# hojinYang/spotify_recSys_challenge_2018

Measured on AMD Instinct MI355X. Metric: playlists scored/sec (encode+decode+top-500) at |vocab|~170k, higher is better.
Workload: dtype f32; 1 GPU; untied DAE scoring: encode+decode(all 170000 cols)+top-500 over 140000 track cols, hidden=256, batch=256/GPU (global 256), ids=zipf, b_dec=zipf, BASELINE.json configs[1]; vocab=170000, n_tracks=140000, hidden=256, global_batch=256, k=500, parallelism=1 GPU, streams=3, decode_gate=True, tau_exchange=False

## Files before the change

include/dae_hip.h:

```cpp
#ifndef DAE_HIP_H
#define DAE_HIP_H

#include <stddef.h>
#include <stdint.h>

#ifdef __cplusplus
extern "C" {
#endif

typedef struct dae_ctx dae_ctx;

#define DAE_OK            0
#define DAE_ERR_ARG      -1
#define DAE_ERR_HIP      -2
#define DAE_ERR_NOMEM    -3
#define DAE_ERR_STATE    -4

#define DAE_OUT_SCORE     0
#define DAE_OUT_LOGIT     1

#define DAE_DTYPE_F32     0
#define DAE_DTYPE_BF16    1
#define DAE_DTYPE_BF16_EXACT 2

// ... 97 lines not shown
                   int k, int out_kind,
                   float* out_score, int32_t* out_idx);

int dae_score_topk_begin(dae_ctx* ctx,
                         const int32_t* row_ptr, const int32_t* col, const float* val,
                         const float* W_enc, const float* b_enc,
                         int V, int H, int B, int dtype, int n_tracks,
                         const int32_t* seed_row_ptr, int k, float* tau_out);
int dae_score_topk_finish(dae_ctx* ctx, const float* tau,
                          const int32_t* seed_row_ptr, const int32_t* seed_col,
                          int out_kind, float* out_score, int32_t* out_idx);

int dae_topk_dense(dae_ctx* ctx, const float* logits, int64_t ld, int B, int ncols, int col_base,
                   const int32_t* seed_row_ptr, const int32_t* seed_col,
                   int k, int out_kind, float* out_score, int32_t* out_idx);

int dae_topk_merge(dae_ctx* ctx, int G, int B, int k,
                   const float* cand_logit, const int32_t* cand_idx,
                   int out_kind, float* out_score, int32_t* out_idx);

int dae_set_overlap_hint(dae_ctx* ctx, int batches_in_flight);

int dae_set_decode_gate(dae_ctx* ctx, void* wait_event, void* record_event);

typedef struct dae_pipeline dae_pipeline;
#define DAE_PIPE_BUSY 1
int dae_pipeline_create(int device, const float* W_enc, const float* b_enc, const float* W_dec, const float* b_dec,
                        int V, int H, int n_tracks, int dtype, int k, int group_rows, int64_t max_nnz, int lanes,
                        int want_scores, int result_blocks, dae_pipeline** out);
int dae_pipeline_destroy(dae_pipeline* p);
int dae_pipeline_submit(dae_pipeline* p, const int64_t* positions, const float* values, int values_broadcast, int64_t nnz,
                        int n_rows, uint64_t* ticket_out);
int dae_pipeline_create_titled(int device, const float* W_enc, const float* b_enc, const float* W_dec, const float* b_dec,
                               int V, int H, int n_tracks, const float* emb, int n_char, int E, const float* conv_w,
                               const float* conv_b, const int32_t* filter_sizes, int n_sizes, int F, const float* Output_WT,
                               const float* Output_b, int ld_feat, int L, int dtype, int k, int group_rows, int64_t max_nnz,
                               int lanes, int want_scores, int result_blocks, dae_pipeline** out);
int dae_pipeline_submit_titled(dae_pipeline* p, const int64_t* positions, const float* values, int values_broadcast, int64_t nnz,
                               int n_rows, const int32_t* titles, const float* titles_use, uint64_t* ticket_out);
int dae_pipeline_flush(dae_pipeline* p);
int dae_pipeline_poll(dae_pipeline* p, int wait, uint64_t* ticket, const int32_t** idx, const float** score, int* n_rows,
                      int* block);
int dae_pipeline_release(dae_pipeline* p, int block);
int dae_pipeline_stats(dae_pipeline* p, uint64_t out3[3]);
int dae_pipeline_times(dae_pipeline* p, uint64_t out4[4]);
int dae_pipeline_exact_margin(dae_pipeline* p, float scale);
// ... 173 lines not shown
```

spotify_recsys_challenge_2018_amd/_lib.py:

```python
import ctypes
import os

_HERE = os.path.dirname(os.path.abspath(__file__))
LIB_PATH = os.path.join(_HERE, "libdae_hip.so")

DAE_OUT_SCORE, DAE_OUT_LOGIT = 0, 1
DAE_MAX_K, DAE_MAX_K_DEEP = 1024, 4096
DAE_DTYPE_F32, DAE_DTYPE_BF16, DAE_DTYPE_BF16_EXACT = 0, 1, 2
DAE_CAND_CHUNK = 256

EXPORTS = [
    "dae_version", "dae_create", "dae_destroy", "dae_set_stream", "dae_last_error",
    "dae_scratch_bytes", "dae_profile_enable", "dae_profile_read", "dae_profile_kernel", "dae_clock_probe", "dae_last_plan",
    "dae_coo_to_csr", "dae_seeds_from_csr", "dae_train_set_create", "dae_train_set_destroy", "dae_train_batch", "dae_train_set_attach_titles", "dae_train_titles", "dae_encode", "dae_prepack_decoder", "dae_prepack_decoder_rows", "dae_share_decoder", "dae_exact_bounds",
    "dae_exact_guard_read", "dae_exact_guard_words", "dae_exact_guard_snapshot", "dae_exact_stats_read", "dae_set_exact_margin", "dae_set_exact_margin_range", "dae_set_exact_audit", "dae_exact_audit_read",
    "dae_set_filter_skip", "dae_filter_skip_read", "dae_filter_skip_last", "dae_tile_bounds_read", "dae_sample_skip_read", "dae_live_proof_read", "dae_last_tau_read", "dae_decode_dense", "dae_decode_topk",
    "dae_score_topk", "dae_score_topk_begin", "dae_score_topk_finish", "dae_topk_dense", "dae_topk_merge", "dae_set_train_dtype", "dae_train_forward_backward",
    "dae_train_shard_encode", "dae_train_shard_decode", "dae_train_shard_finish", "dae_title_features", "dae_title_prepack_features",
    "dae_mix_scores", "dae_decode_mix_term", "dae_set_score_mix", "dae_decode_mix_term_add", "dae_ensemble_topk", "dae_mix_topk_exact", "dae_mix_exact_shape_ok", "dae_title_score_exact", "dae_title_score", "dae_row_sums", "dae_mix_weights", "dae_title_loss_backward", "dae_title_loss_backward_cols", "dae_title_conv_backward", "dae_adam_step",
    "dae_adam_rows_begin", "dae_adam_rows_apply", "dae_adam_rows_flush", "dae_set_enc_grad_prezeroed",
    "dae_arm_decoder_adam", "dae_set_decode_gate", "dae_set_overlap_hint",
    "dae_pipeline_create", "dae_pipeline_create_titled", "dae_pipeline_destroy", "dae_pipeline_submit", "dae_pipeline_submit_titled", "dae_pipeline_flush", "dae_pipeline_poll",
    "dae_pipeline_release", "dae_pipeline_stats", "dae_pipeline_exact_margin", "dae_pipeline_times", "dae_pipeline_last_error",
    "dae_rank_metrics", "dae_pipeline_enable_eval", "dae_pipeline_submit_eval", "dae_pipeline_poll_eval",
    "dae_decode_candidates", "dae_score_candidates", "dae_mix_candidates", "dae_rank_candidates",
    "dae_rank_of_plan", "dae_decode_rank_of", "dae_score_rank_of", "dae_mix_rank_of",
    "dae_catalogue_create", "dae_catalogue_destroy", "dae_prepack_decoder_catalogue", "dae_score_topk_catalogue",
    "dae_decode_topk_catalogue", "dae_title_score_catalogue", "dae_pipeline_set_catalogue",
]
DAE_PIPE_BUSY = 1

_lib = None


class DaeError(RuntimeError):
    pass


def load():
    global _lib
    if _lib is not None:
        return _lib
    if not os.path.exists(LIB_PATH):
        raise DaeError(
# ... 71 lines not shown
    lib.dae_decode_mix_term_add.argtypes = lib.dae_decode_mix_term.argtypes
    lib.dae_ensemble_topk.argtypes = [ctypes.POINTER(vp), c_int, ctypes.POINTER(vp), ctypes.POINTER(c_int), ctypes.POINTER(vp),
                                      vp, vp, c_int, vp, c_int, c_int, c_int, vp, vp, c_int, vp, vp]
    lib.dae_mix_topk_exact.argtypes = [vp, vp, vp, c_i64, vp, c_i64, c_int, vp, vp, c_int, vp, vp, c_int, vp, vp, vp]
    lib.dae_mix_exact_shape_ok.argtypes = [c_int, c_int]
    lib.dae_row_sums.argtypes = [vp, vp, vp, vp, c_int, c_f, c_u32, vp]
    lib.dae_title_score_exact.argtypes = [vp, vp, vp, vp, c_int, c_i64, c_int, c_int, vp, vp, c_int, vp, c_int, vp, c_int, c_int, vp, vp,
                                          ctypes.POINTER(ctypes.c_int32), c_int, c_int, c_int, vp, c_int, c_int, vp, vp, vp, vp]
    lib.dae_mix_weights.argtypes = [vp, vp, vp, vp, c_int, c_f, c_u32, vp, vp, vp]
    lib.dae_title_loss_backward.argtypes = [vp, vp, c_i64, vp, c_i64, vp, vp, vp, vp, vp, c_int, c_int, c_int,
                                            vp, c_int, vp, vp, vp, vp, vp]
    lib.dae_title_loss_backward_cols.argtypes = [vp, vp, c_i64, vp, c_i64, vp, vp, vp, vp, vp, c_int, c_int, c_int, c_int,
                                                 vp, c_int, vp, vp, vp, vp, vp]
    lib.dae_title_conv_backward.argtypes = [vp, vp, c_int, c_int, vp, c_int, c_int, vp, ctypes.POINTER(ctypes.c_int32),
                                            c_int, c_int, vp, vp, vp, c_i64, c_f, c_u32, vp, vp, vp]
    lib.dae_adam_step.argtypes = [vp, vp, vp, vp, vp, c_i64, c_f, c_f, c_f, c_f, c_int]
    lib.dae_adam_rows_begin.argtypes = [vp, vp, vp, vp, vp, vp, c_int, c_int, c_int, vp, vp, c_int, c_f, c_f, c_f, c_int]
    lib.dae_adam_rows_apply.argtypes = [vp, vp, vp, vp, vp, vp, vp, c_int, c_int, c_int, vp, vp, c_int,
                                        c_f, c_f, c_f, c_f, c_int]
    lib.dae_adam_rows_flush.argtypes = [vp, vp, vp, vp, vp, vp, c_int, c_int, c_int, c_f, c_f, c_f, c_int]
    lib.dae_set_enc_grad_prezeroed.argtypes = [vp, c_int]
    lib.dae_arm_decoder_adam.argtypes = [vp, vp, vp, c_f, c_f, c_f, c_f, c_int]
    lib.dae_set_decode_gate.argtypes = [vp, vp, vp]
    lib.dae_set_overlap_hint.argtypes = [vp, c_int]
    u64p, i32pp, f32pp, ip = (ctypes.POINTER(ctypes.c_uint64), ctypes.POINTER(ctypes.POINTER(ctypes.c_int32)),
                              ctypes.POINTER(ctypes.POINTER(ctypes.c_float)), ctypes.POINTER(c_int))
    lib.dae_pipeline_create.argtypes = [c_int, vp, vp, vp, vp, c_int, c_int, c_int, c_int, c_int, c_int, c_i64, c_int, c_int, c_int,
                                        ctypes.POINTER(vp)]
    i32p = ctypes.POINTER(ctypes.c_int32)
    lib.dae_pipeline_create_titled.argtypes = ([c_int, vp, vp, vp, vp, c_int, c_int, c_int,
                                                vp, c_int, c_int, vp, vp, i32p, c_int, c_int,
                                                vp, vp, c_int, c_int] +
                                               [c_int] * 3 + [c_i64] + [c_int] * 3 + [ctypes.POINTER(vp)])
    lib.dae_pipeline_submit_titled.argtypes = [vp, vp, vp, c_int, c_i64, c_int, vp, vp, u64p]
    lib.dae_title_score.argtypes = [vp, vp, c_int, vp, vp, c_int, c_i64, c_int, c_int, vp, vp, c_int, vp, c_int, vp, c_int, c_int, vp, vp,
                                    i32p, c_int, c_int, c_int, vp, c_int, c_int, vp, vp, vp, vp]
    lib.dae_pipeline_destroy.argtypes = [vp]
    lib.dae_pipeline_submit.argtypes = [vp, vp, vp, c_int, c_i64, c_int, u64p]
    lib.dae_pipeline_flush.argtypes = [vp]
    lib.dae_pipeline_poll.argtypes = [vp, c_int, u64p, i32pp, f32pp, ip, ip]
    lib.dae_pipeline_release.argtypes = [vp, c_int]
    lib.dae_pipeline_stats.argtypes = [vp, u64p]
    lib.dae_pipeline_exact_margin.argtypes = [vp, c_f]
    lib.dae_pipeline_times.argtypes = [vp, u64p]
    lib.dae_pipeline_last_error.argtypes = [vp]
    lib.dae_rank_metrics.argtypes = [vp, vp, c_i64, c_int, c_int, vp, vp, vp, vp]
# ... 197 lines not shown
        return "f32" if int(dtype) == DAE_DTYPE_F32 else "bf16"

    def _drop_share(self, dtype):
        self.__dict__.setdefault("_shares", {}).pop(self._slot(dtype), None)

    def prepack_decoder_rows(self, W_rows, b_rows, col_lo, dtype=DAE_DTYPE_F32):
        n, H = W_rows.shape
        assert W_rows.is_contiguous() and b_rows.is_contiguous() and b_rows.numel() == n
        self.check(self.lib.dae_prepack_decoder_rows(self.h, _ptr(W_rows), _ptr(b_rows), int(n), H, int(col_lo), int(dtype)))
        self._drop_share(dtype)

    def title_loss_backward_cols(self, z_title, dae_score, y_csr, w_title, w_playlist, col_lo, col_hi, n_batch, feat,
                                 Output_WT_rows, gOutput_WT_rows, gOutput_b_rows, dfeat_partial, cost_partial):
        B, ld = feat.shape
        self.check(self.lib.dae_title_loss_backward_cols(
            self.h, _ptr(z_title), int(z_title.stride(0)), _ptr(dae_score), int(dae_score.stride(0)),
            _ptr(y_csr[0]), _ptr(y_csr[1]), _ptr(y_csr[2]), _ptr(w_title), _ptr(w_playlist), int(B), int(col_lo), int(col_hi),
            int(n_batch), _ptr(feat), int(ld), _ptr(Output_WT_rows), _ptr(gOutput_WT_rows), _ptr(gOutput_b_rows),
            _ptr(dfeat_partial), _ptr(cost_partial)))

    def set_overlap_hint(self, batches_in_flight):
        self.check(self.lib.dae_set_overlap_hint(self.h, int(batches_in_flight)))

    def share_decoder(self, src, dtype=DAE_DTYPE_F32):
        self.check(self.lib.dae_share_decoder(self.h, src.h, int(dtype)))
        self.__dict__.setdefault("_shares", {})[self._slot(dtype)] = src

    def exact_bounds(self, eps_out):
        self.check(self.lib.dae_exact_bounds(self.h, _ptr(eps_out)))

    def set_exact_margin(self, scale):
        self.check(self.lib.dae_set_exact_margin(self.h, float(scale)))
        self._exact_margin = float(scale)

    def set_exact_margin_range(self, col_from, col_to, scale):
        self.check(self.lib.dae_set_exact_margin_range(self.h, int(col_from), int(col_to), float(scale)))

    def set_exact_audit(self, every_n, n_tiles=16):
        self.check(self.lib.dae_set_exact_audit(self.h, int(every_n), int(n_tiles)))

    def exact_audit_read(self):
        a = (ctypes.c_uint64 * 3)()
        self.check(self.lib.dae_exact_audit_read(self.h, a))
        return {"audits": int(a[0]), "checked": int(a[1]), "violations": int(a[2])}

    def exact_guard_read(self):
# ... 540 lines not shown
```

spotify_recsys_challenge_2018_amd/csrc/api.hip:

```cpp
#include <stdarg.h>

#include <climits>

#include "dae_internal.h"

thread_local std::string g_dae_create_err;

int dae_fail(dae_ctx* ctx, int code, const char* fmt, ...)
{
    char buf[512];
    va_list ap;
    va_start(ap, fmt);
    vsnprintf(buf, sizeof(buf), fmt, ap);
    va_end(ap);
    if (ctx) ctx->err = buf; else g_dae_create_err = buf;
    return code;
}

int dae_reserve(dae_ctx* ctx, dae_buf& b, size_t bytes)
{
    if (bytes <= b.bytes && b.p) return DAE_OK;
    if (bytes == 0) bytes = 16;
    if (b.p) {
        hipError_t e = hipStreamSynchronize(ctx->stream);
// ... 24 lines not shown
extern "C" {

int dae_version(void) { return 1002; }

int dae_create(int device, dae_ctx** out)
{
    if (!out) return dae_fail(nullptr, DAE_ERR_ARG, "out is null");
    int n = 0;
    hipError_t e = hipGetDeviceCount(&n);
    if (e != hipSuccess || n <= 0)
        return dae_fail(nullptr, DAE_ERR_HIP, "no HIP device available (%s)", hipGetErrorString(e));
    if (device < 0 || device >= n)
        return dae_fail(nullptr, DAE_ERR_ARG, "device %d out of range [0,%d)", device, n);
    e = hipSetDevice(device);
    if (e != hipSuccess) return dae_fail(nullptr, DAE_ERR_HIP, "hipSetDevice: %s", hipGetErrorString(e));
    hipDeviceProp_t prop;
    e = hipGetDeviceProperties(&prop, device);
    if (e != hipSuccess) return dae_fail(nullptr, DAE_ERR_HIP, "hipGetDeviceProperties: %s", hipGetErrorString(e));
    if (strncmp(prop.gcnArchName, "gfx950", 6) != 0)
        return dae_fail(nullptr, DAE_ERR_HIP, "device %d is %s; this library is built for gfx950 only",
                        device, prop.gcnArchName);
    dae_ctx* c = new dae_ctx();
    c->device = device;
    *out = c;
    return DAE_OK;
}

int dae_destroy(dae_ctx* ctx)
{
    if (!ctx) return DAE_OK;
    (void)hipSetDevice(ctx->device);
    (void)hipStreamSynchronize(ctx->stream);
    auto release = [](dae_buf& b) { if (b.p) (void)hipFree(b.p); };
    for (dae_packed* pk : {&ctx->pk_f32, &ctx->pk_bf16}) {
        if (!pk->borrowed) dae_packed_shared_bufs(*pk, release);
        release(pk->order); release(pk->ident);
    }
    for (dae_buf* b : {&ctx->h_packed, &ctx->sample, &ctx->tau, &ctx->sample_top, &ctx->cand, &ctx->cand_cnt, &ctx->gmax,
                       &ctx->h_packed16, &ctx->h_scratch, &ctx->train_a, &ctx->train_b, &ctx->train_c, &ctx->train_d, &ctx->csr_tmp,
                       &ctx->feed_tmp, &ctx->row_bad, &ctx->guard, &ctx->refined, &ctx->refstat, &ctx->mix_fhat, &ctx->title_scratch,
                       &ctx->tile_band, &ctx->title_tab, &ctx->audit, &ctx->audit_stat, &ctx->title_y1, &ctx->live, &ctx->skip_stat, &ctx->live_sync,
                       &ctx->row_d, &ctx->samp_tab, &ctx->sskip_stat,
                       &ctx->cand_list, &ctx->cat_seeds, &ctx->rank_of})
        release(*b);
    for (hipEvent_t ev : ctx->prof_ev) (void)hipEventDestroy(ev);
    delete ctx;
    return DAE_OK;
}

int dae_set_stream(dae_ctx* ctx, void* hip_stream)
{
    if (!ctx) return DAE_ERR_ARG;
    ctx->stream = static_cast<hipStream_t>(hip_stream);
    return DAE_OK;
}

const char* dae_last_error(const dae_ctx* ctx)
{
    return ctx ? ctx->err.c_str() : g_dae_create_err.c_str();
}

size_t dae_scratch_bytes(const dae_ctx* ctx) { return ctx ? ctx->scratch_total : 0; }

int dae_profile_enable(dae_ctx* ctx, int on)
{
    if (!ctx) return DAE_ERR_ARG;
    ctx->prof_on = on != 0;
    ctx->prof_used = 0;
// ... 95 lines not shown
    if (!pk.borrowed) return;
    dae_packed_shared_bufs(pk, [](dae_buf& b) { b = dae_buf{}; });
    pk.borrowed = false; pk.valid = false; pk.exact = false; pk.order_nrank = -1;
}

int dae_share_decoder(dae_ctx* dst, const dae_ctx* src, int dtype)
{
    if (!dst) return DAE_ERR_ARG;
    if (!src || src == dst) return dae_fail(dst, DAE_ERR_ARG, "dae_share_decoder: needs another context");
    if (dst->device != src->device) return dae_fail(dst, DAE_ERR_ARG, "dae_share_decoder: contexts on different devices");
    if (!dae_known_dtype(dtype)) return dae_fail(dst, DAE_ERR_ARG, "unknown dtype %d", dtype);
    const dae_packed& sp = dtype == DAE_DTYPE_F32 ? src->pk_f32 : src->pk_bf16;
    dae_packed& dp = dtype == DAE_DTYPE_F32 ? dst->pk_f32 : dst->pk_bf16;
    if (!sp.valid || (dtype == DAE_DTYPE_BF16_EXACT && !sp.exact))
        return dae_fail(dst, DAE_ERR_STATE, "dae_share_decoder: the source context holds no such image");
    if (sp.borrowed) return dae_fail(dst, DAE_ERR_ARG, "dae_share_decoder: share from the context that owns the image");
    if (!dp.borrowed) {
        hipError_t e = hipStreamSynchronize(dst->stream);
        if (e != hipSuccess) return dae_fail(dst, DAE_ERR_HIP, "sync: %s", hipGetErrorString(e));
        dae_packed_shared_bufs(dp, [&](dae_buf& b) {
            if (b.p) { (void)hipFree(b.p); dst->scratch_total -= b.bytes; b = dae_buf{}; }
        });
    }
    const dae_buf order = dp.order, ident = dp.ident;
    dp = sp;
    dp.order = order; dp.ident = ident; dp.order_nrank = -1; dp.order_nsamp = -1;
    dp.borrowed = true;
    int rc = dae_reserve(dst, dp.ident, (size_t)(dp.ntiles > 0 ? dp.ntiles : 1) * sizeof(int));
    if (rc) return rc;
    return dae_launch_tile_iota(dst, static_cast<int*>(dp.ident.p), dp.ntiles);
}

int dae_prepack_decoder(dae_ctx* ctx, const float* W_dec, const float* b_dec, int V, int H,
                        int col_lo, int col_hi, int dtype)
{
    if (!ctx) return DAE_ERR_ARG;
    if (!W_dec || !b_dec) return dae_fail(ctx, DAE_ERR_ARG, "null pointer");
    if (H <= 0 || V <= 0 || col_lo < 0 || col_hi > V || col_lo >= col_hi)
        return dae_fail(ctx, DAE_ERR_ARG, "bad shape V=%d H=%d cols=[%d,%d)", V, H, col_lo, col_hi);
    unborrow(dtype == DAE_DTYPE_F32 ? ctx->pk_f32 : ctx->pk_bf16);
    if (dtype == DAE_DTYPE_F32) return dae_launch_prepack_f32(ctx, W_dec, b_dec, V, H, col_lo, col_hi);
    if (dtype == DAE_DTYPE_BF16) return dae_launch_prepack_bf16(ctx, W_dec, b_dec, V, H, col_lo, col_hi);
    if (dtype == DAE_DTYPE_BF16_EXACT) return dae_launch_prepack_bf16(ctx, W_dec, b_dec, V, H, col_lo, col_hi, 1);
    return dae_fail(ctx, DAE_ERR_ARG, "unknown dtype %d", dtype);
}

int dae_prepack_decoder_rows(dae_ctx* ctx, const float* W_rows, const float* b_rows, int n_rows, int H, int col_lo,
                             int dtype)
{
    if (!ctx) return DAE_ERR_ARG;
    if (!W_rows || !b_rows) return dae_fail(ctx, DAE_ERR_ARG, "null pointer");
    if (n_rows <= 0 || H <= 0 || col_lo < 0 || (int64_t)col_lo + n_rows > INT_MAX)
        return dae_fail(ctx, DAE_ERR_ARG, "bad shape n_rows=%d H=%d col_lo=%d", n_rows, H, col_lo);
    const float* W = W_rows - (size_t)col_lo * H;
    const float* b = b_rows - (size_t)col_lo;
    return dae_prepack_decoder(ctx, W, b, col_lo + n_rows, H, col_lo, col_lo + n_rows, dtype);
}

int dae_exact_bounds(dae_ctx* ctx, float* eps_out)
{
    if (!ctx) return DAE_ERR_ARG;
    if (!eps_out) return dae_fail(ctx, DAE_ERR_ARG, "null pointer");
    const dae_packed& pk = ctx->pk_bf16;
// ... 364 lines not shown
                            float keep_prob, uint32_t seed, float* g_emb, float* g_conv_w, float* g_conv_b)
{
    if (!ctx) return DAE_ERR_ARG;
    if (!titles || !emb || !conv_w || !filter_sizes || !argmax || !feat_raw || !dfeat || !g_emb || !g_conv_w || !g_conv_b)
        return dae_fail(ctx, DAE_ERR_ARG, "null pointer");
    if (B <= 0) return DAE_OK;
    if (!(keep_prob > 0.f && keep_prob <= 1.f)) return dae_fail(ctx, DAE_ERR_ARG, "keep probability must be in (0,1]");
    return dae_launch_title_conv_backward(ctx, titles, B, L, emb, n_char, E, conv_w, filter_sizes, n_sizes, F, argmax,
                                          feat_raw, dfeat, ld, keep_prob, seed, g_emb, g_conv_w, g_conv_b);
}

int dae_set_overlap_hint(dae_ctx* ctx, int batches_in_flight)
{
    if (!ctx) return DAE_ERR_ARG;
    ctx->overlap_hint = batches_in_flight > 1 ? 1 : 0;
    return DAE_OK;
}

int dae_set_decode_gate(dae_ctx* ctx, void* wait_event, void* record_event)
{
    if (!ctx) return DAE_ERR_ARG;
    ctx->gate_wait = static_cast<hipEvent_t>(wait_event);
    ctx->gate_record = static_cast<hipEvent_t>(record_event);
    return DAE_OK;
}

int dae_set_enc_grad_prezeroed(dae_ctx* ctx, int on)
{
    if (!ctx) return DAE_ERR_ARG;
    ctx->enc_grad_prezeroed = on ? 1 : 0;
    return DAE_OK;
}

}
```

spotify_recsys_challenge_2018_amd/csrc/dae_internal.h:

```cpp
#pragma once
#include <hip/hip_runtime.h>
#include <hip/hip_ext.h>
#include <stdint.h>
#include <stdio.h>
#include <stdlib.h>
#include <string.h>
#include <string>
#include <unordered_set>
#include <vector>

#include "../../include/dae_hip.h"
#include "score_plan.h"
#include "mix_plan.h"
#include "tau_search.h"
#include "empty_proof.h"

constexpr int DAE_TITLE_MAX_SIZES = 8;
constexpr int DAE_VT = 32;
constexpr int DAE_HPAD = 32;
constexpr int DAE_REFINED_CAP = 4096;
constexpr size_t DAE_GUARD_BYTES = 2 * sizeof(int);

struct dae_buf {
    void* p = nullptr;
    size_t bytes = 0;
};

struct dae_packed {
    bool valid = false;
    bool borrowed = false;
    int V = 0, H = 0, Hp = 0;
    int col_lo = 0, col_hi = 0;
    int ntiles = 0;
    dae_buf W;
    dae_buf bias;
    dae_buf tile_ub; bool ub_valid = false;
    dae_buf bias16;
    dae_buf order;
// ... 36 lines not shown
    hipStream_t stream = nullptr;
    std::string err;
    size_t scratch_total = 0;

    dae_packed pk_f32, pk_bf16;

    dae_buf h_packed;
    dae_buf h_packed16;
    dae_buf h_scratch;
    long long h_geom_key = -1;
    void* h_geom_ptr = nullptr;
    long long h16_geom_key = -1;
    void* h16_geom_ptr = nullptr;
    dae_buf sample;
    dae_buf gmax;
    dae_buf tau;
    dae_buf sample_top;
    dae_buf cand;
    dae_buf cand_cnt;
    dae_buf train_a, train_b, train_c, train_d;
    float* arm_m = nullptr; float* arm_v = nullptr; float arm_alpha = 0.f, arm_b1 = 0.f, arm_b2 = 0.f, arm_eps = 0.f;
    const float* mixT = nullptr; int64_t mix_ld = 0; const float* mix_w = nullptr; int mix_ncols = 0;
    hipEvent_t gate_wait = nullptr, gate_record = nullptr;
    int enc_grad_prezeroed = 0;
    int adam_t = 0; float adam_b1 = 0.f, adam_b2 = 0.f, adam_b1p = 1.f, adam_b2p = 1.f;
    int train_dtype = DAE_DTYPE_F32;
    dae_buf csr_tmp;
    dae_buf feed_tmp;
    dae_topk_state tk;
    int overlap_hint = 0;
    dae_buf row_bad;
    dae_buf refined;
    dae_buf refstat; int refstat_rows = 0;
    dae_buf guard;
    float exact_margin = 1.0f;
    int margin_lo = 0, margin_hi = 0; float margin_scale = 1.0f;
    int audit_every = 64, audit_tiles = 16;
    uint64_t audit_seq = 0, audits_run = 0;
    dae_buf title_y1;
    dae_buf audit_stat;
    dae_buf audit;
    dae_buf mix_fhat;
    dae_buf title_scratch;
    dae_buf title_tab; const float* ttab_emb = nullptr; const float* ttab_w = nullptr; int ttab_nchar = 0, ttab_E = 0, ttab_F = 0,
        ttab_nsizes = 0; int ttab_fs[DAE_TITLE_MAX_SIZES] = {0};
    dae_buf tile_band; long long band_gen = -1; int band_nsamp = 0, band_nbrg = 0, band_waves = 0;
// ... 152 lines not shown
    int mode;
    const int* list;
};
constexpr int DAE_SSKIP_SLOTS = 2 * DAE_NUM_CU;
constexpr int DAE_SSKIP_PAIRS = DAE_SSKIP_SLOTS / DAE_NUM_XCD;
struct dae_sample_skip {
    const float2* ub;
    const float* beta; int n_beta;
    const float* mu;
    const float* row_d;
    const int32_t* seed_row_ptr; int k;
    unsigned long long* stat;
    unsigned* tab;
    float2* pair;
};
int dae_launch_decode_dense_f32(dae_ctx* ctx, const dae_rowgeom& g, int B, const dae_tileset& ts,
                                int apply_sigmoid, int mask_from_col, float* out, int64_t ld,
                                int fill_pad, int dtype = DAE_DTYPE_F32, float* gmax = nullptr,
                                int64_t ld_gmax = 0, int gmax_per_wave = 0, int bias_sel = 0,
                                const dae_sample_skip* skip = nullptr);
int dae_launch_decode_filter_f32(dae_ctx* ctx, const dae_rowgeom& g, int B, const dae_tileset& ts,
                                 const float* tau, int n_valid_col, uint2* cand, int* cand_cnt,
                                 int cap, int dtype = DAE_DTYPE_F32, int bias_sel = 0, const int* live_cnt = nullptr,
                                 const int* live_list = nullptr);

int dae_launch_decode_scaled_T(dae_ctx* ctx, const dae_rowgeom& g, int B, const dae_tileset& ts, const float* row_scale,
                               float* outT, int64_t ldT, int dtype = DAE_DTYPE_F32, bool add = false);

int dae_launch_decode_loss_f32(dae_ctx* ctx, const dae_rowgeom& g, int B, float inv_n_batch,
                               float* dzT, int64_t ldT, float* loss_part, int dtype = DAE_DTYPE_F32,
                               int dz16 = 0);

int dae_launch_decode_loss_rowmajor(dae_ctx* ctx, const dae_rowgeom& g, int B, int V, int H, const float* W,
                                    const float* bias, const float* h, float inv_n_batch, float* dzT, int64_t ldT,
                                    float* loss_part);

int dae_launch_decode_loss_dh(dae_ctx* ctx, const dae_rowgeom& g, int B, int V, int H, const float* W, const float* bias,
                              const float* h, float inv_n_batch, float* dzT, int64_t ldT, float* loss_part, float* part, int Bpad64);

struct dae_decp;
int dae_launch_decode_generic(dae_ctx* ctx, int epi, int dt, const dae_rowgeom& g, const dae_decp& p);
int dae_launch_decode_gmax_half(dae_ctx* ctx, const dae_rowgeom& g, const dae_decp& p);

int dae_train_step_f32(dae_ctx* ctx,
        const int32_t* x_row_ptr, const int32_t* x_col, const float* x_val,
        const int32_t* y_row_ptr, const int32_t* y_col, const float* y_val,
        const float* W_enc, const float* b_enc, const float* W_dec, const float* b_dec,
// ... 174 lines not shown
```

spotify_recsys_challenge_2018_amd/csrc/decode_common.h:

```cpp
#pragma once
#include "dae_internal.h"

typedef float f32x16 __attribute__((ext_vector_type(16)));
typedef __bf16 bf16x8 __attribute__((ext_vector_type(8)));
typedef float f32x2_t __attribute__((ext_vector_type(2)));
typedef __bf16 bf16x2_t __attribute__((ext_vector_type(2)));

template <int N> struct IntC { static constexpr int value = N; };

__device__ __forceinline__ bf16x8 as_bf16x8(const uint4 u) { return __builtin_bit_cast(bf16x8, u); }

__device__ __forceinline__ float dae_bf16_value(float f) { return __uint_as_float(dae_bf16_rne(f) << 16); }

__device__ __forceinline__ unsigned pk_bf16(float a, float b)
{
    const f32x2_t v = {a, b};
    return __builtin_bit_cast(unsigned, __builtin_convertvector(v, bf16x2_t));
}

constexpr int DT_F32 = 0;
constexpr int DT_BF16 = 1;

__device__ __forceinline__ uint4 bf16_ones_fragment(int hi)
{
// ... 1 lines not shown
}

constexpr int EPI_DENSE = 0;
constexpr int EPI_FILTER = 1;
constexpr int EPI_LOSS = 2;
constexpr int EPI_GMAX = 3;
constexpr int EPI_TERM_ADD = 4;

struct dae_decp {
    const float4* Wp;
    const float* bias;
    const uint4* bias16;
    const float4* hp;
    int G;
    int ncols;
    int col_lo;
    int B, n_rg, nb_rg, Bpad;
    dae_tileset ts;
    float* out; int64_t ld; int apply_sigmoid; int mask_from_col; int fill_pad; int vec_ok;
    float* gmax; int64_t ld_gmax;
    int gmax_per_wave;
    const float* tau; int n_valid_col; uint2* cand; int* cand_cnt; int cap;
    const int* live_cnt; const int* live_list;
    dae_sample_skip sk;
    float* outT; int64_t ld_outT; const float* row_scale;
    const float* mixT; int64_t mix_ld; const float* mix_w; int mix_ncols;
    float inv_nb; float* dzT; int64_t ldT; float* loss_part;
    int dz16;
};

template <class T>
__device__ __forceinline__ T dae_max_nan(T a, T b) { return (a != a) ? a : ((b > a || b != b) ? b : a); }
template <class T>
__device__ __forceinline__ T dae_min_nan(T a, T b) { return -dae_max_nan(-a, -b); }

__device__ __forceinline__ bool dae_tile_is_live(float A_t, float M_t, double d_max, float tau_min)
{
    const double d = d_max * (1.0 + 0x1p-40);
    const double A = (double)A_t, dm = d * (double)M_t;
    const double U = A + dm + (fabs(A) + fabs(dm)) * 0x1p-48;
    return !(U < (double)tau_min);
}

__device__ __forceinline__ void dae_edge_tile_bound(const float* tile_ub, int ntiles, int nrank, int lane, float& ea, float& em)
{
    const int t_edge = nrank >> 5;
// ... 38 lines not shown
```

spotify_recsys_challenge_2018_amd/csrc/decode_f32.hip:

```cpp
#include <climits>

#include "decode_common.h"

namespace {

struct LossRmP {
    const float* W; const float* bias; const float* h;
    int V, H, B, n_rg, nb_rg;
    float inv_nb; float* dzT; int64_t ldT; float* loss_part;
};

__global__ __launch_bounds__(512, 1) void decode_loss_dh_bf16_kernel(const LossRmP p, float* __restrict__ part, int Bpad64)
{
    constexpr int NW = 8, LDW = 132, LDT = 18;
    extern __shared__ __attribute__((aligned(16))) unsigned dyn[];
    unsigned* const wt = dyn;
    unsigned* const wt2 = dyn + 2 * 32 * LDW;
    uint4* const hq = reinterpret_cast<uint4*>(dyn + 2 * 32 * LDW + 2 * 256 * LDT);
    float* const wsum = reinterpret_cast<float*>(hq + 8 * 8 * 64);
    const int tid = threadIdx.x, lane = tid & 63, hi = lane >> 5, j = lane & 31;
    const int wave = __builtin_amdgcn_readfirstlane(tid >> 6);
    const int row = wave * 32 + j;
    const int H4 = p.H >> 2;
    const float4* W4 = reinterpret_cast<const float4*>(p.W);
// ... 293 lines not shown
}
#undef K5F_LOAD
#undef K5F_STAGE

template <int DUMMY>
__global__ __launch_bounds__(256, 1) void decode_f32_h256_filter_kernel(const dae_decp p)
{
    constexpr int RB = 4, G = 32, NW = 4, R_TILE = 128;
    extern __shared__ __attribute__((aligned(16))) float4 lds4[];
    const int tid = threadIdx.x;
    const int lane = tid & 63;
    const int wave = __builtin_amdgcn_readfirstlane(tid >> 6);
    const int hi = lane >> 5;
    const int j = lane & 31;

    const int gs = DAE_NUM_XCD * p.n_rg;
    const int q = blockIdx.x / gs, rem_b = blockIdx.x % gs;
    const int rg = rem_b / DAE_NUM_XCD;
    const int bir = q * DAE_NUM_XCD + (rem_b % DAE_NUM_XCD);

    constexpr int n_h4 = RB * 64 * G;
    const int* const tlist = p.live_cnt ? p.live_list + (size_t)rg * p.ts.n_items : p.ts.list;
    const int n_items = p.live_cnt ? __builtin_amdgcn_readfirstlane(p.live_cnt[rg]) : p.ts.n_items;
    if (n_items <= 0) {
        if (tid < R_TILE) p.cand_cnt[(size_t)bir * p.Bpad + rg * R_TILE + tid] = 0;
        return;
    }
    const int n_ws = p.nb_rg * NW;
    const int ws = wave * p.nb_rg + bir;
    const int R = n_items / n_ws, rem = n_items - R * n_ws;
    const bool split = rem > 0 && 2 * rem <= n_ws;
    const int n_it = R + (ws < (split ? 2 * rem : rem) ? 1 : 0);
    auto item_at = [&](int r) {
        r = r < n_it - 1 ? r : n_it - 1;
        r = r < 0 ? 0 : r;
        const int it = r < R ? ws + r * n_ws : R * n_ws + (split ? (ws >> 1) : ws);
        return it < n_items ? it : 0;
    };
    const int tv_cur = tlist[item_at(0)], tv_nxt = tlist[item_at(1)];
    {
        const float4* src = p.hp + (size_t)rg * n_h4;
        constexpr int NT = NW * 64;
#pragma unroll
        for (int i0 = 0; i0 < n_h4; i0 += 8 * NT) {
            float4 v[8];
#pragma unroll
            for (int u = 0; u < 8; ++u) v[u] = src[i0 + u * NT + tid];
#pragma unroll
            for (int u = 0; u < 8; ++u) lds4[i0 + u * NT + tid] = v[u];
        }
    }
    int* lcnt = reinterpret_cast<int*>(lds4 + n_h4);
    float* ltau = reinterpret_cast<float*>(lcnt + R_TILE);
    if (tid < R_TILE) {
        lcnt[tid] = 0;
        ltau[tid] = rg * R_TILE + tid < p.B ? p.tau[rg * R_TILE + tid] : __builtin_inff();
    }
    float4 wb0, wb1, wb2, wb3;
    float4 bA[RB], bB[RB];
    int t_cur = __builtin_amdgcn_readfirstlane(tv_cur), t_nxt = __builtin_amdgcn_readfirstlane(tv_nxt);
    {
        const float4* w0 = p.Wp + (size_t)t_cur * G * 64 + lane;
        wb0 = w0[0]; wb1 = w0[64]; wb2 = w0[128]; wb3 = w0[192];
    }
    __syncthreads();

    float tau_r[RB];
#pragma unroll
    for (int rb = 0; rb < RB; ++rb) tau_r[rb] = ltau[rb * 32 + j];
#pragma unroll
    for (int rb = 0; rb < RB; ++rb) bA[rb] = lds4[rb * 64 + lane];

    for (int r = 0; r < n_it; ++r) {
        const int t = t_cur;
// ... 566 lines not shown
    p.inv_nb = inv_n_batch; p.dzT = dzT; p.ldT = ldT; p.loss_part = loss_part;
    const size_t lds = ((size_t)2 * 32 * 132 + (size_t)2 * 256 * 18) * 4 + (size_t)8 * 8 * 64 * 16 + 64;
    DAE_HIP_CHECK(ctx, dae_lds_limit_once(ctx, &decode_loss_dh_bf16_kernel, lds));
    hipLaunchKernelGGL(decode_loss_dh_bf16_kernel, dim3(g.grid), dim3(512), lds, ctx->stream, p, part, Bpad64);
    DAE_CHECK_LAUNCH(ctx, "decode_loss_dh_bf16_kernel");
    return DAE_OK;
}

int dae_launch_decode_loss_f32(dae_ctx* ctx, const dae_rowgeom& g, int B, float inv_n_batch,
                               float* dzT, int64_t ldT, float* loss_part, int dtype, int dz16)
{
    dae_decp p;
    const dae_packed& pk = dtype == DAE_DTYPE_F32 ? ctx->pk_f32 : ctx->pk_bf16;
    dae_tileset ts{pk.ntiles, 1, 0, static_cast<const int*>(pk.ident.p)};
    int rc = fill_common(ctx, g, B, ts, p, dtype);
    if (rc) return rc;
    p.dzT = dzT; p.ldT = ldT; p.loss_part = loss_part; p.inv_nb = inv_n_batch;
    p.dz16 = (dtype == DAE_DTYPE_BF16 && dz16) ? 1 : 0;
    return dae_launch_decode_generic(ctx, EPI_LOSS, dtype == DAE_DTYPE_BF16 ? DT_BF16 : DT_F32, g, p);
}

int dae_launch_decode_filter_f32(dae_ctx* ctx, const dae_rowgeom& g, int B, const dae_tileset& ts,
                                 const float* tau, int n_valid_col, uint2* cand, int* cand_cnt,
                                 int cap, int dtype, int bias_sel, const int* live_cnt, const int* live_list)
{
    dae_decp p;
    int rc = fill_common(ctx, g, B, ts, p, dtype, bias_sel);
    if (rc) return rc;
    p.tau = tau; p.n_valid_col = n_valid_col; p.cand = cand; p.cand_cnt = cand_cnt; p.cap = cap;
    if (live_cnt && !dae_filter_takes_live(g, dtype, p.G * DAE_KG, p.mixT != nullptr))
        return dae_fail(ctx, DAE_ERR_ARG, "live tile lists: the fp32 hidden-256 filter launch only");
    p.live_cnt = live_cnt; p.live_list = live_list;
    if (dae_filter_takes_live(g, dtype, p.G * DAE_KG, p.mixT != nullptr)) {
        const size_t lds = (size_t)4 * 64 * 32 * sizeof(float4) + 128 * sizeof(int) + 128 * sizeof(float);
        DAE_HIP_CHECK(ctx, dae_lds_limit_once(ctx, &decode_f32_h256_filter_kernel<0>, 160 * 1024));
        hipEvent_t e0 = nullptr, e1 = nullptr;
        dae_take_profile_events(ctx, "decode_f32_h256_filter_kernel<0>", e0, e1);
        hipExtLaunchKernelGGL(decode_f32_h256_filter_kernel<0>, dim3(g.grid), dim3(256), lds, ctx->stream, e0, e1, 0, p);
        DAE_CHECK_LAUNCH(ctx, "decode_f32_h256_filter_kernel");
        return DAE_OK;
    }
    if (bf16_fast_filter(g, dtype, p.G) && !p.mixT) {
        const size_t lds = (size_t)(g.R_TILE / 32) * 64 * 16 * sizeof(float4) + (size_t)g.R_TILE * (sizeof(int) + sizeof(float)) + 16;
        DAE_HIP_CHECK(ctx, dae_lds_limit_once(ctx, &decode_bf16_h256_filter_kernel<1, 4, 8, 8>, 160 * 1024));
        hipEvent_t e0 = nullptr, e1 = nullptr;
        dae_take_profile_events(ctx, "decode_bf16_h256_filter_kernel<1, 4, 8, 8>", e0, e1);
        hipExtLaunchKernelGGL((decode_bf16_h256_filter_kernel<1, 4, 8, 8>), dim3(g.grid), dim3(512), lds,
                              ctx->stream, e0, e1, 0, p);
        DAE_CHECK_LAUNCH(ctx, "decode_bf16_h256_filter_kernel");
        return DAE_OK;
    }
    return dae_launch_decode_generic(ctx, EPI_FILTER, dtype == DAE_DTYPE_F32 ? DT_F32 : DT_BF16, g, p);
}
```

spotify_recsys_challenge_2018_amd/csrc/score.hip:

```cpp
#include <climits>

#include "dae_internal.h"

namespace {

thread_local int32_t g_last_plan[8] = {0, 0, 0, 0, 0, 0, 0, 0};

int prof_begin(dae_ctx* ctx)
{
    if (!ctx->prof_on) return DAE_OK;
    if (ctx->prof_used + 2 > ctx->prof_ev.size()) {
        for (int i = 0; i < 2; ++i) {
            hipEvent_t ev;
            DAE_HIP_CHECK(ctx, hipEventCreate(&ev));
            ctx->prof_ev.push_back(ev);
        }
    }
    ctx->prof_armed = true;
    return DAE_OK;
}

dae_rowgeom geom_for(int dtype, int B, int Hp)
{
    return dtype == DAE_DTYPE_F32 ? dae_row_geometry(B, Hp) : dae_row_geometry_bf16(B, Hp);
}

int hidden_pads_zeroed(dae_ctx* ctx, long long& key, void*& ptr, const dae_buf& img, size_t bytes, int B, int H, int R_TILE)
{
    const long long want = ((long long)B << 32) | ((long long)H << 12) | (long long)R_TILE;
    if (key == want && ptr == img.p) return DAE_OK;
    if (bytes) DAE_HIP_CHECK(ctx, hipMemsetAsync(img.p, 0, bytes, ctx->stream));
    key = want; ptr = img.p;
    return DAE_OK;
}

int reserve_row_d(dae_ctx* ctx, const dae_rowgeom& g)
{
    ctx->row_d_fresh = false;
    return dae_reserve(ctx, ctx->row_d, (size_t)g.Bpad * 4 * sizeof(float));
}

// ... 265 lines not shown
    if (!pl.fused) {
        dae_dense_src ds{static_cast<const float*>(ctx->sample.p), pl.ld_s, (int)pl.ld_s, pk->col_lo, 1, nullptr};
        return dae_launch_topk_dense(ctx, ds, ta);
    }

    const int n_filter = pl.n_filter, cap = pl.cap;
    rc = dae_reserve(ctx, ctx->cand, (size_t)g.nb_rg * g.Bpad * cap * sizeof(uint2));
    if (rc) return rc;
    rc = dae_reserve(ctx, ctx->cand_cnt, (size_t)g.nb_rg * g.Bpad * sizeof(int));
    if (rc) return rc;
    dae_tileset tsB{n_filter, pl.S, 3, pl.whole_b ? tk.order : tk.order + pl.n_samp};
    const int* live_cnt = nullptr; const int* live_list = nullptr;
    if (pl.build_live) {
        int* lc; int* ll;
        rc = reserve_live(ctx, g, n_filter, &lc, &ll);
        if (rc) return rc;
        if (!tk.live_built) {
            rc = dae_launch_live_tiles(ctx, *pk, g, B, tsB.list, n_filter, tau_src, pl.nrank, lc, ll,
                                       static_cast<unsigned long long*>(ctx->skip_stat.p));
            if (rc) return rc;
        }
        live_cnt = lc; live_list = ll; ctx->live_n_rg = g.n_rg;
    }
    if (ctx->gate_wait) DAE_HIP_CHECK(ctx, hipStreamWaitEvent(ctx->stream, ctx->gate_wait, 0));
    rc = prof_begin(ctx); if (rc) return rc;
    rc = dae_launch_decode_filter_f32(ctx, g, B, tsB, tau_src, pl.n_valid_col, static_cast<uint2*>(ctx->cand.p),
                                      static_cast<int*>(ctx->cand_cnt.p), cap, dtype, pl.exact ? 2 : 0, live_cnt, live_list);
    if (rc) return rc;
    ctx->prof_armed = false;
    if (ctx->gate_record) DAE_HIP_CHECK(ctx, hipEventRecord(ctx->gate_record, ctx->stream));

    dae_pair_group g0{static_cast<const uint2*>(ctx->sample_top.p), tk.sample_cnt, 0, pl.ld_s, 0, 1, 0};
    dae_pair_group g1{static_cast<const uint2*>(ctx->cand.p), static_cast<const int*>(ctx->cand_cnt.p),
                      (int64_t)g.Bpad * cap, cap, g.Bpad, g.nb_rg, 0};
    if (pl.exact) {
        rc = dae_ensure_guard(ctx);
        if (rc) return rc;
        dae_exact_src xs{h32, (int64_t)pk->H, pk->H, static_cast<const float*>(pk->W32.p),
                         static_cast<const float*>(pk->bias.p), pk->col_lo, row_bad,
                         static_cast<const float*>(pk->eps.p) + (size_t)pk->ntiles * 32,
                         static_cast<const float*>(pk->eps.p), static_cast<int*>(ctx->guard.p)};
        rc = dae_reserve(ctx, ctx->refined, (size_t)g.Bpad * DAE_REFINED_CAP * sizeof(uint2) + (size_t)g.Bpad * sizeof(int));
        if (rc) return rc;
        uint2* rf = static_cast<uint2*>(ctx->refined.p);
        int* rf_cnt = reinterpret_cast<int*>(rf + (size_t)g.Bpad * DAE_REFINED_CAP);
        rc = dae_reserve(ctx, ctx->refstat, (size_t)g.Bpad * 2 * sizeof(int));
        if (rc) return rc;
        ctx->refstat_rows = B;
        const bool fuse = dae_exact_refine_can_fuse(ta);
        rc = dae_launch_exact_refine(ctx, g1, xs, B, k, seed_row_ptr, rf, rf_cnt, DAE_REFINED_CAP, static_cast<int*>(ctx->refstat.p),
                                     fuse ? &ta : nullptr);
        if (!rc && ctx->audit_every > 0 && ctx->audit_tiles > 0 && (++ctx->audit_seq % (uint64_t)ctx->audit_every) == 0)
            rc = dae_launch_exact_audit(ctx, g, B, xs, pl.nrank, ctx->audit_tiles);
// ... 411 lines not shown
```

Baseline: 9.859 million playlists/s.

## Skip decode-gate stream wait/record when device feedback reports no live tiles

Adds an adaptive policy for the cross-stream decode gate. Block 0 of the filter kernel writes its call number and the summed live-tile count into host-mapped coherent memory. On later calls the host reads that word and skips the hipStreamWaitEvent/hipEventRecord pair once two consecutive fresh observations count as light. With the light threshold at 0/1, only calls with zero live tiles qualify, so on typical inputs the gate still fires while the kernel now also does a host-memory write every call. The policy can be overridden through an environment variable or a new API call, and counters are exposed for inspection.

```diff
diff --git a/include/dae_hip.h b/include/dae_hip.h
--- a/include/dae_hip.h
+++ b/include/dae_hip.h
@@ -143,6 +143,9 @@
 int dae_set_overlap_hint(dae_ctx* ctx, int batches_in_flight);
 
 int dae_set_decode_gate(dae_ctx* ctx, void* wait_event, void* record_event);
+int dae_set_gate_policy(dae_ctx* ctx, int mode);
+int dae_gate_read(dae_ctx* ctx, uint64_t out3[3]);
+int dae_gate_feedback_peek(dae_ctx* ctx, uint64_t* word_out, int* allocated_out);
 
 typedef struct dae_pipeline dae_pipeline;
 #define DAE_PIPE_BUSY 1
diff --git a/spotify_recsys_challenge_2018_amd/_lib.py b/spotify_recsys_challenge_2018_amd/_lib.py
--- a/spotify_recsys_challenge_2018_amd/_lib.py
+++ b/spotify_recsys_challenge_2018_amd/_lib.py
@@ -19,7 +19,7 @@
     "dae_train_shard_encode", "dae_train_shard_decode", "dae_train_shard_finish", "dae_title_features", "dae_title_prepack_features",
     "dae_mix_scores", "dae_decode_mix_term", "dae_set_score_mix", "dae_decode_mix_term_add", "dae_ensemble_topk", "dae_mix_topk_exact", "dae_mix_exact_shape_ok", "dae_title_score_exact", "dae_title_score", "dae_row_sums", "dae_mix_weights", "dae_title_loss_backward", "dae_title_loss_backward_cols", "dae_title_conv_backward", "dae_adam_step",
     "dae_adam_rows_begin", "dae_adam_rows_apply", "dae_adam_rows_flush", "dae_set_enc_grad_prezeroed",
-    "dae_arm_decoder_adam", "dae_set_decode_gate", "dae_set_overlap_hint",
+    "dae_arm_decoder_adam", "dae_set_decode_gate", "dae_set_gate_policy", "dae_gate_read", "dae_gate_feedback_peek", "dae_set_overlap_hint",
     "dae_pipeline_create", "dae_pipeline_create_titled", "dae_pipeline_destroy", "dae_pipeline_submit", "dae_pipeline_submit_titled", "dae_pipeline_flush", "dae_pipeline_poll",
     "dae_pipeline_release", "dae_pipeline_stats", "dae_pipeline_exact_margin", "dae_pipeline_times", "dae_pipeline_last_error",
     "dae_rank_metrics", "dae_pipeline_enable_eval", "dae_pipeline_submit_eval", "dae_pipeline_poll_eval",
@@ -137,6 +137,9 @@
     lib.dae_set_enc_grad_prezeroed.argtypes = [vp, c_int]
     lib.dae_arm_decoder_adam.argtypes = [vp, vp, vp, c_f, c_f, c_f, c_f, c_int]
     lib.dae_set_decode_gate.argtypes = [vp, vp, vp]
+    lib.dae_set_gate_policy.argtypes = [vp, c_int]
+    lib.dae_gate_read.argtypes = [vp, ctypes.POINTER(ctypes.c_uint64)]
+    lib.dae_gate_feedback_peek.argtypes = [vp, ctypes.POINTER(ctypes.c_uint64), ctypes.POINTER(c_int)]
     lib.dae_set_overlap_hint.argtypes = [vp, c_int]
     u64p, i32pp, f32pp, ip = (ctypes.POINTER(ctypes.c_uint64), ctypes.POINTER(ctypes.POINTER(ctypes.c_int32)),
                               ctypes.POINTER(ctypes.POINTER(ctypes.c_float)), ctypes.POINTER(c_int))
@@ -380,6 +383,24 @@
     def set_overlap_hint(self, batches_in_flight):
         self.check(self.lib.dae_set_overlap_hint(self.h, int(batches_in_flight)))
 
+    def set_decode_gate(self, wait_event=None, record_event=None):
+        ev = [ctypes.c_void_p(e.cuda_event) if e is not None else None for e in (wait_event, record_event)]
+        self.check(self.lib.dae_set_decode_gate(self.h, ev[0], ev[1]))
+
+    def set_gate_policy(self, mode):
+        self.check(self.lib.dae_set_gate_policy(self.h, int(mode)))
+
+    def gate_read(self):
+        a = (ctypes.c_uint64 * 3)()
+        self.check(self.lib.dae_gate_read(self.h, a))
+        return {"calls": int(a[0]), "waits": int(a[1]), "records": int(a[2])}
+
+    def gate_feedback_peek(self):
+        w, alloc = ctypes.c_uint64(0), ctypes.c_int(0)
+        self.check(self.lib.dae_gate_feedback_peek(self.h, ctypes.byref(w), ctypes.byref(alloc)))
+        word = None if w.value == 2 ** 64 - 1 else (int(w.value >> 32), int(w.value & 0xFFFFFFFF))
+        return word, bool(alloc.value)
+
     def share_decoder(self, src, dtype=DAE_DTYPE_F32):
         self.check(self.lib.dae_share_decoder(self.h, src.h, int(dtype)))
         self.__dict__.setdefault("_shares", {})[self._slot(dtype)] = src
diff --git a/spotify_recsys_challenge_2018_amd/csrc/api.hip b/spotify_recsys_challenge_2018_amd/csrc/api.hip
--- a/spotify_recsys_challenge_2018_amd/csrc/api.hip
+++ b/spotify_recsys_challenge_2018_amd/csrc/api.hip
@@ -70,6 +70,8 @@
                         device, prop.gcnArchName);
     dae_ctx* c = new dae_ctx();
     c->device = device;
+    if (const char* gp = getenv("DAE_GATE_POLICY"))
+        if ((gp[0] == '0' || gp[0] == '1' || gp[0] == '2') && gp[1] == 0) c->gate_policy = gp[0] - '0';
     *out = c;
     return DAE_OK;
 }
@@ -92,6 +94,7 @@
                        &ctx->cand_list, &ctx->cat_seeds, &ctx->rank_of})
         release(*b);
     for (hipEvent_t ev : ctx->prof_ev) (void)hipEventDestroy(ev);
+    if (ctx->gate_fb) (void)hipHostFree(ctx->gate_fb);
     delete ctx;
     return DAE_OK;
 }
@@ -233,6 +236,7 @@
             if (b.p) { (void)hipFree(b.p); dst->scratch_total -= b.bytes; b = dae_buf{}; }
         });
     }
+    dst->gate_state = dae_gate_state{};
     const dae_buf order = dp.order, ident = dp.ident;
     dp = sp;
     dp.order = order; dp.ident = ident; dp.order_nrank = -1; dp.order_nsamp = -1;
@@ -250,6 +254,7 @@
     if (H <= 0 || V <= 0 || col_lo < 0 || col_hi > V || col_lo >= col_hi)
         return dae_fail(ctx, DAE_ERR_ARG, "bad shape V=%d H=%d cols=[%d,%d)", V, H, col_lo, col_hi);
     unborrow(dtype == DAE_DTYPE_F32 ? ctx->pk_f32 : ctx->pk_bf16);
+    ctx->gate_state = dae_gate_state{};
     if (dtype == DAE_DTYPE_F32) return dae_launch_prepack_f32(ctx, W_dec, b_dec, V, H, col_lo, col_hi);
     if (dtype == DAE_DTYPE_BF16) return dae_launch_prepack_bf16(ctx, W_dec, b_dec, V, H, col_lo, col_hi);
     if (dtype == DAE_DTYPE_BF16_EXACT) return dae_launch_prepack_bf16(ctx, W_dec, b_dec, V, H, col_lo, col_hi, 1);
@@ -660,6 +665,33 @@
     if (!ctx) return DAE_ERR_ARG;
     ctx->gate_wait = static_cast<hipEvent_t>(wait_event);
     ctx->gate_record = static_cast<hipEvent_t>(record_event);
+    ctx->gate_state = dae_gate_state{};
+    return DAE_OK;
+}
+
+int dae_set_gate_policy(dae_ctx* ctx, int mode)
+{
+    if (!ctx) return DAE_ERR_ARG;
+    if (mode != DAE_GATE_POLICY_AUTO && mode != DAE_GATE_POLICY_ALWAYS && mode != DAE_GATE_POLICY_NEVER)
+        return dae_fail(ctx, DAE_ERR_ARG, "dae_set_gate_policy: mode %d is none of 0 (auto), 1 (always), 2 (never)", mode);
+    ctx->gate_policy = mode;
+    return DAE_OK;
+}
+
+int dae_gate_read(dae_ctx* ctx, uint64_t out3[3])
+{
+    if (!ctx) return DAE_ERR_ARG;
+    if (!out3) return dae_fail(ctx, DAE_ERR_ARG, "null pointer");
+    for (int i = 0; i < 3; ++i) { out3[i] = ctx->gate_stat[i]; ctx->gate_stat[i] = 0; }
+    return DAE_OK;
+}
+
+int dae_gate_feedback_peek(dae_ctx* ctx, uint64_t* word_out, int* allocated_out)
+{
+    if (!ctx) return DAE_ERR_ARG;
+    if (!word_out || !allocated_out) return dae_fail(ctx, DAE_ERR_ARG, "null pointer");
+    *word_out = ctx->gate_fb ? __atomic_load_n(ctx->gate_fb, __ATOMIC_RELAXED) : DAE_GATE_WORD_NONE;
+    *allocated_out = ctx->gate_fb ? 1 : 0;
     return DAE_OK;
 }
 
diff --git a/spotify_recsys_challenge_2018_amd/csrc/dae_internal.h b/spotify_recsys_challenge_2018_amd/csrc/dae_internal.h
--- a/spotify_recsys_challenge_2018_amd/csrc/dae_internal.h
+++ b/spotify_recsys_challenge_2018_amd/csrc/dae_internal.h
@@ -14,6 +14,7 @@
 #include "mix_plan.h"
 #include "tau_search.h"
 #include "empty_proof.h"
+#include "gate_policy.h"
 
 constexpr int DAE_TITLE_MAX_SIZES = 8;
 constexpr int DAE_VT = 32;
@@ -96,6 +97,11 @@
     float* arm_m = nullptr; float* arm_v = nullptr; float arm_alpha = 0.f, arm_b1 = 0.f, arm_b2 = 0.f, arm_eps = 0.f;
     const float* mixT = nullptr; int64_t mix_ld = 0; const float* mix_w = nullptr; int mix_ncols = 0;
     hipEvent_t gate_wait = nullptr, gate_record = nullptr;
+    int gate_policy = DAE_GATE_POLICY_AUTO;
+    dae_gate_state gate_state;
+    uint64_t* gate_fb = nullptr; unsigned long long* gate_fb_dev = nullptr;
+    uint32_t gate_call = 0;
+    uint64_t gate_stat[3] = {0, 0, 0};
     int enc_grad_prezeroed = 0;
     int adam_t = 0; float adam_b1 = 0.f, adam_b2 = 0.f, adam_b1p = 1.f, adam_b2p = 1.f;
     int train_dtype = DAE_DTYPE_F32;
@@ -294,7 +300,7 @@
 int dae_launch_decode_filter_f32(dae_ctx* ctx, const dae_rowgeom& g, int B, const dae_tileset& ts,
                                  const float* tau, int n_valid_col, uint2* cand, int* cand_cnt,
                                  int cap, int dtype = DAE_DTYPE_F32, int bias_sel = 0, const int* live_cnt = nullptr,
-                                 const int* live_list = nullptr);
+                                 const int* live_list = nullptr, unsigned long long* gate_fb = nullptr, uint32_t gate_call = 0);
 
 int dae_launch_decode_scaled_T(dae_ctx* ctx, const dae_rowgeom& g, int B, const dae_tileset& ts, const float* row_scale,
                                float* outT, int64_t ldT, int dtype = DAE_DTYPE_F32, bool add = false);
diff --git a/spotify_recsys_challenge_2018_amd/csrc/decode_common.h b/spotify_recsys_challenge_2018_amd/csrc/decode_common.h
--- a/spotify_recsys_challenge_2018_amd/csrc/decode_common.h
+++ b/spotify_recsys_challenge_2018_amd/csrc/decode_common.h
@@ -47,6 +47,7 @@
     int gmax_per_wave;
     const float* tau; int n_valid_col; uint2* cand; int* cand_cnt; int cap;
     const int* live_cnt; const int* live_list;
+    unsigned long long* gate_fb; unsigned gate_call;
     dae_sample_skip sk;
     float* outT; int64_t ld_outT; const float* row_scale;
     const float* mixT; int64_t mix_ld; const float* mix_w; int mix_ncols;
diff --git a/spotify_recsys_challenge_2018_amd/csrc/decode_f32.hip b/spotify_recsys_challenge_2018_amd/csrc/decode_f32.hip
--- a/spotify_recsys_challenge_2018_amd/csrc/decode_f32.hip
+++ b/spotify_recsys_challenge_2018_amd/csrc/decode_f32.hip
@@ -339,8 +339,17 @@
     constexpr int n_h4 = RB * 64 * G;
     const int* const tlist = p.live_cnt ? p.live_list + (size_t)rg * p.ts.n_items : p.ts.list;
     const int n_items = p.live_cnt ? __builtin_amdgcn_readfirstlane(p.live_cnt[rg]) : p.ts.n_items;
+    auto report_live = [&]() {
+        if (blockIdx.x == 0 && wave == 0 && p.gate_fb) {
+            int live = lane < p.n_rg ? p.live_cnt[lane] : 0;
+#pragma unroll
+            for (int d = 32; d >= 1; d >>= 1) live += __shfl_xor(live, d);
+            if (lane == 0) *p.gate_fb = ((unsigned long long)p.gate_call << 32) | (unsigned long long)(unsigned)live;
+        }
+    };
     if (n_items <= 0) {
         if (tid < R_TILE) p.cand_cnt[(size_t)bir * p.Bpad + rg * R_TILE + tid] = 0;
+        report_live();
         return;
     }
     const int n_ws = p.nb_rg * NW;
@@ -367,6 +376,7 @@
             for (int u = 0; u < 8; ++u) lds4[i0 + u * NT + tid] = v[u];
         }
     }
+    report_live();
     int* lcnt = reinterpret_cast<int*>(lds4 + n_h4);
     float* ltau = reinterpret_cast<float*>(lcnt + R_TILE);
     if (tid < R_TILE) {
@@ -979,7 +989,8 @@
 
 int dae_launch_decode_filter_f32(dae_ctx* ctx, const dae_rowgeom& g, int B, const dae_tileset& ts,
                                  const float* tau, int n_valid_col, uint2* cand, int* cand_cnt,
-                                 int cap, int dtype, int bias_sel, const int* live_cnt, const int* live_list)
+                                 int cap, int dtype, int bias_sel, const int* live_cnt, const int* live_list,
+                                 unsigned long long* gate_fb, uint32_t gate_call)
 {
     dae_decp p;
     int rc = fill_common(ctx, g, B, ts, p, dtype, bias_sel);
@@ -988,6 +999,9 @@
     if (live_cnt && !dae_filter_takes_live(g, dtype, p.G * DAE_KG, p.mixT != nullptr))
         return dae_fail(ctx, DAE_ERR_ARG, "live tile lists: the fp32 hidden-256 filter launch only");
     p.live_cnt = live_cnt; p.live_list = live_list;
+    if (gate_fb && (!live_cnt || g.n_rg > 64))
+        return dae_fail(ctx, DAE_ERR_ARG, "gate feedback: a launch with live lists of at most 64 row groups only");
+    p.gate_fb = gate_fb; p.gate_call = gate_call;
     if (dae_filter_takes_live(g, dtype, p.G * DAE_KG, p.mixT != nullptr)) {
         const size_t lds = (size_t)4 * 64 * 32 * sizeof(float4) + 128 * sizeof(int) + 128 * sizeof(float);
         DAE_HIP_CHECK(ctx, dae_lds_limit_once(ctx, &decode_f32_h256_filter_kernel<0>, 160 * 1024));
diff --git a/spotify_recsys_challenge_2018_amd/csrc/gate_policy.h b/spotify_recsys_challenge_2018_amd/csrc/gate_policy.h
--- /dev/null
+++ b/spotify_recsys_challenge_2018_amd/csrc/gate_policy.h
@@ -0,0 +1,49 @@
+#pragma once
+#include <stdint.h>
+
+constexpr uint64_t DAE_GATE_WORD_NONE = ~(uint64_t)0;
+constexpr uint32_t DAE_GATE_STALE_CALLS = 8;
+constexpr int DAE_GATE_RUN = 2;
+constexpr uint64_t DAE_GATE_LIGHT_NUM = 0, DAE_GATE_LIGHT_DEN = 1;
+
+constexpr int DAE_GATE_POLICY_AUTO = 0;
+constexpr int DAE_GATE_POLICY_ALWAYS = 1;
+constexpr int DAE_GATE_POLICY_NEVER = 2;
+
+struct dae_gate_state {
+    uint32_t since_reset = 0;
+    uint32_t last_call = 0;
+    bool has_last = false;
+    int run = 0;
+};
+
+struct dae_gate_decision {
+    bool issue;
+    dae_gate_state next;
+};
+
+inline bool dae_gate_is_light(uint64_t live_tiles, uint64_t planned_tiles)
+{
+    return live_tiles * DAE_GATE_LIGHT_DEN <= planned_tiles * DAE_GATE_LIGHT_NUM;
+}
+
+inline dae_gate_decision dae_gate_decide(const dae_gate_state& s, uint64_t word, uint32_t call_no, uint64_t planned_tiles)
+{
+    dae_gate_decision d{true, s};
+    dae_gate_state& n = d.next;
+    if (n.since_reset != UINT32_MAX) n.since_reset += 1;
+    const uint32_t obs_call = (uint32_t)(word >> 32);
+    const uint32_t age = call_no - obs_call;
+    const bool fresh = word != DAE_GATE_WORD_NONE && age >= 1 && age <= DAE_GATE_STALE_CALLS && age <= s.since_reset;
+    if (!fresh) {
+        n.run = 0; n.has_last = false;
+        return d;
+    }
+    if (!(s.has_last && s.last_call == obs_call)) {
+        n.has_last = true; n.last_call = obs_call;
+        if (!dae_gate_is_light(word & 0xFFFFFFFFu, planned_tiles)) n.run = 0;
+        else if (n.run < DAE_GATE_RUN) n.run += 1;
+    }
+    d.issue = n.run < DAE_GATE_RUN;
+    return d;
+}
diff --git a/spotify_recsys_challenge_2018_amd/csrc/score.hip b/spotify_recsys_challenge_2018_amd/csrc/score.hip
--- a/spotify_recsys_challenge_2018_amd/csrc/score.hip
+++ b/spotify_recsys_challenge_2018_amd/csrc/score.hip
@@ -17,6 +17,22 @@
         }
     }
     ctx->prof_armed = true;
+    return DAE_OK;
+}
+
+int gate_feedback_block(dae_ctx* ctx)
+{
+    if (ctx->gate_fb) return DAE_OK;
+    void* host = nullptr; void* dev = nullptr;
+    DAE_HIP_CHECK(ctx, hipHostMalloc(&host, 64, hipHostMallocMapped | hipHostMallocCoherent));
+    *static_cast<uint64_t*>(host) = DAE_GATE_WORD_NONE;
+    hipError_t e = hipHostGetDevicePointer(&dev, host, 0);
+    if (e != hipSuccess) {
+        (void)hipHostFree(host);
+        return dae_fail(ctx, DAE_ERR_HIP, "hipHostGetDevicePointer failed: %s", hipGetErrorString(e));
+    }
+    ctx->gate_fb = static_cast<uint64_t*>(host);
+    ctx->gate_fb_dev = static_cast<unsigned long long*>(dev);
     return DAE_OK;
 }
 
@@ -328,13 +344,36 @@
         }
         live_cnt = lc; live_list = ll; ctx->live_n_rg = g.n_rg;
     }
-    if (ctx->gate_wait) DAE_HIP_CHECK(ctx, hipStreamWaitEvent(ctx->stream, ctx->gate_wait, 0));
+    unsigned long long* fb_dev = nullptr;
+    bool gate = ctx->gate_wait || ctx->gate_record;
+    if (gate) {
+        ctx->gate_stat[0] += 1;
+        ctx->gate_call += 1;
+        if (live_cnt && g.n_rg <= 64) {
+            rc = gate_feedback_block(ctx);
+            if (rc) return rc;
+            fb_dev = ctx->gate_fb_dev;
+            const dae_gate_decision gd = dae_gate_decide(ctx->gate_state, __atomic_load_n(ctx->gate_fb, __ATOMIC_RELAXED),
+                                                         ctx->gate_call, (uint64_t)n_filter * (uint64_t)g.n_rg);
+            ctx->gate_state = gd.next;
+            if (ctx->gate_policy == DAE_GATE_POLICY_AUTO) gate = gd.issue;
+        }
+        if (ctx->gate_policy == DAE_GATE_POLICY_NEVER) gate = false;
+    }
+    if (gate && ctx->gate_wait) {
+        DAE_HIP_CHECK(ctx, hipStreamWaitEvent(ctx->stream, ctx->gate_wait, 0));
+        ctx->gate_stat[1] += 1;
+    }
     rc = prof_begin(ctx); if (rc) return rc;
     rc = dae_launch_decode_filter_f32(ctx, g, B, tsB, tau_src, pl.n_valid_col, static_cast<uint2*>(ctx->cand.p),
-                                      static_cast<int*>(ctx->cand_cnt.p), cap, dtype, pl.exact ? 2 : 0, live_cnt, live_list);
+                                      static_cast<int*>(ctx->cand_cnt.p), cap, dtype, pl.exact ? 2 : 0, live_cnt, live_list,
+                                      fb_dev, ctx->gate_call);
     if (rc) return rc;
     ctx->prof_armed = false;
-    if (ctx->gate_record) DAE_HIP_CHECK(ctx, hipEventRecord(ctx->gate_record, ctx->stream));
+    if (gate && ctx->gate_record) {
+        DAE_HIP_CHECK(ctx, hipEventRecord(ctx->gate_record, ctx->stream));
+        ctx->gate_stat[2] += 1;
+    }
 
     dae_pair_group g0{static_cast<const uint2*>(ctx->sample_top.p), tk.sample_cnt, 0, pl.ld_s, 0, 1, 0};
     dae_pair_group g1{static_cast<const uint2*>(ctx->cand.p), static_cast<const int*>(ctx->cand_cnt.p),
```

Result: no change. 9.790 million playlists/s (-0.7%).
